# vsois/hanabi-agents

Measured on AMD Instinct MI355X. Metric: env_steps_per_sec, higher is better.
Workload: dtype u8 env/encoder + bfloat16 Q-net GEMM (fp32 accumulate, fp32 master weights)

## Files before the change

### hanabi-agents_amd/csrc/actor_fused.hip

```cpp
#include <hip/hip_runtime.h>
#include <hip/hip_bf16.h>
#include <hip/hip_fp16.h>

#include <cstdint>
#include <type_traits>

#include "../../include/hanabi_hip.h"
#include "common.hpp"
#include "env_kernel.hpp"

using hb::fail;

namespace {

typedef __bf16 bf16x8 __attribute__((ext_vector_type(8)));
typedef _Float16 f16x8 __attribute__((ext_vector_type(8)));
typedef float f32x4 __attribute__((ext_vector_type(4)));

constexpr int FM = 128;
constexpr int FH = 512;
constexpr int FNT = 512;
constexpr int FK = 51;
constexpr int S2 = FH / 32;
constexpr int LUT_BYTES = 65536;
constexpr int H_BYTES = FM * FH * 2;
constexpr int FRAG_FLOATS = 3 * 8 * FM;
constexpr int LDS_TOTAL = H_BYTES + FRAG_FLOATS * 4;
constexpr float NEG_BIG = -1e30f;

struct FusedArgs {
  const uint32_t* obs;
  long long m;
  int words;
  int s1;
  const uint4* w1f;
  const float* b1;
  const uint4* w2f;
  const float* b2;
  const float* support;
  float* q;
  int n_actions, n_pass;
  const int8_t* legal;
  int32_t* actions;
  float epsilon;
  unsigned long long seed, draw;
  long long first_gid;
  unsigned long long* stamps;
};

#ifdef HB_STAMPS
#define HB_FSTAMP(slot)                                                                              \
  do {                                                                                               \
    __builtin_amdgcn_sched_barrier(0);                                                               \
    unsigned long long hb_t_;                                                                        \
    asm volatile("s_memtime %0\n\ts_waitcnt lgkmcnt(0)" : "=s"(hb_t_)::"memory");                    \
    if (a.stamps && lane == 0) a.stamps[(static_cast<long long>(blockIdx.x) * 8 + wave) * 16 + (slot)] = hb_t_; \
    __builtin_amdgcn_sched_barrier(0);                                                               \
  } while (0)
#define HB_FSTAMP_REAL(slot)                                                                         \
  do {                                                                                               \
    unsigned long long hb_t_;                                                                        \
    asm volatile("s_memrealtime %0\n\ts_waitcnt lgkmcnt(0)" : "=s"(hb_t_)::"memory");                \
    if (a.stamps && lane == 0) a.stamps[(static_cast<long long>(blockIdx.x) * 8 + wave) * 16 + (slot)] = hb_t_; \
  } while (0)
#else
#define HB_FSTAMP(slot) do {} while (0)
#define HB_FSTAMP_REAL(slot) do {} while (0)
#endif

template <bool F16>
__device__ __forceinline__ uint32_t pack16(float lo, float hi) {
  if constexpr (F16) {
    const _Float16 a = static_cast<_Float16>(lo), b = static_cast<_Float16>(hi);
    uint16_t ua, ub;
    __builtin_memcpy(&ua, &a, 2);
    __builtin_memcpy(&ub, &b, 2);
    return static_cast<uint32_t>(ua) | (static_cast<uint32_t>(ub) << 16);
  } else {
    const __hip_bfloat16 a = __float2bfloat16(lo), b = __float2bfloat16(hi);
    return static_cast<uint32_t>(*reinterpret_cast<const uint16_t*>(&a)) |
           (static_cast<uint32_t>(*reinterpret_cast<const uint16_t*>(&b)) << 16);
  }
}
template <bool F16>
__device__ __forceinline__ uint32_t bits2_one(uint32_t b, int p) {
  const uint32_t t = (b >> (2 * p)) & 3u;
  return __umul24((t | (t << 15)) & 0x00010001u, F16 ? 0x3C00u : 0x3F80u);
}
template <bool F16>
__device__ __forceinline__ f32x4 mfma16(const uint4& wv, const uint4& xv, const f32x4& c) {
  if constexpr (F16) {
    union { uint4 u; f16x8 f; } w, x;
    w.u = wv; x.u = xv;
    return __builtin_amdgcn_mfma_f32_16x16x32_f16(w.f, x.f, c, 0, 0, 0);
  } else {
    union { uint4 u; bf16x8 f; } w, x;
    w.u = wv; x.u = xv;
    return __builtin_amdgcn_mfma_f32_16x16x32_bf16(w.f, x.f, c, 0, 0, 0);
  }
}
typedef float f32x2 __attribute__((ext_vector_type(2)));
typedef unsigned int u32x2 __attribute__((ext_vector_type(2)));
__device__ __forceinline__ float vmax(float a, float b) {
  float r;
  asm("v_max_f32 %0, %1, %2" : "=v"(r) : "v"(a), "v"(b));
  return r;
}
__device__ __forceinline__ float vmax3(float a, float b, float c) {
  float r;
  asm("v_max3_f32 %0, %1, %2, %3" : "=v"(r) : "v"(a), "v"(b), "v"(c));
  return r;
}
__device__ __forceinline__ float exp2_fast(float x) { return __builtin_amdgcn_exp2f(x); }

template <bool F16, class K, int EG>
__device__ __forceinline__ void actor_fused_body(const FusedArgs& a) {
  __shared__ __attribute__((aligned(16))) unsigned char lds[LDS_TOTAL];
  const int tid = threadIdx.x, lane = tid & 63;
  const int wave = __builtin_amdgcn_readfirstlane(tid >> 6);
  const int r = lane & 15, qd = lane >> 4;
  const long long row0 = static_cast<long long>(blockIdx.x) * FM;
  const int s1 = a.s1, G = (s1 + 3) >> 2;
  unsigned char* lutb = lds + (LDS_TOTAL - LUT_BYTES);
  const int bits_off = LDS_TOTAL - LUT_BYTES - 2048 * G;
  unsigned char* bits = lds + bits_off;
  const int m_early = bits_off >> 14;

  HB_FSTAMP_REAL(14);
  HB_FSTAMP(0);
  const uint4* w1p = a.w1f + (4 * wave) * 64 + lane;
  uint4 wa[4], wb[4];
#pragma unroll
  for (int n = 0; n < 4; ++n) wa[n] = w1p[n * 64];

  uint32_t w[4] = {0u, 0u, 0u, 0u};
  auto load_item = [&](int it) {
    const int rr = it & (FM - 1), g = it >> 7;
    long long row = row0 + rr;
    if (row >= a.m) row = a.m - 1;
    const uint32_t* src = a.obs + row * a.words + 4 * g;
#pragma unroll
    for (int i = 0; i < 4; ++i) w[i] = (4 * g + i < a.words) ? src[i] : 0u;
  };
  if (tid < FM * G) load_item(tid);
  for (int e = tid; e < 4096; e += FNT) {
    const uint32_t v = static_cast<uint32_t>(e) >> 4;
    *reinterpret_cast<uint4*>(lutb + e * 16) = make_uint4(bits2_one<F16>(v, 0), bits2_one<F16>(v, 1), bits2_one<F16>(v, 2), bits2_one<F16>(v, 3));
  }
  for (int it = tid; it < FM * G; it += FNT) {
    const int rr = it & (FM - 1), g = it >> 7;
    if (it != tid) load_item(it);
    uint32_t* dst = reinterpret_cast<uint32_t*>(bits) + (static_cast<size_t>((rr >> 4) * G + g) * 64 + (rr & 15));
#pragma unroll
    for (int qq = 0; qq < 4; ++qq) {
      const uint32_t o = ((w[0] >> (8 * qq)) & 0xFFu) | (((w[1] >> (8 * qq)) & 0xFFu) << 8) | (((w[2] >> (8 * qq)) & 0xFFu) << 16) |
                         (((w[3] >> (8 * qq)) & 0xFFu) << 24);
      dst[qq * 16] = o;
    }
  }
  HB_FSTAMP(1);
  __syncthreads();
  HB_FSTAMP(2);

  f32x4 acc[4][8];
#pragma unroll
  for (int n = 0; n < 4; ++n) {
// ... 211 lines not shown
#pragma unroll
    HB_M HB_SWAP16(tF[m], HB_ADD)
#pragma unroll
    HB_M HB_SWAP16(zs[m], HB_ADD)
#pragma unroll
    HB_M HB_SWAP16(zt[m], HB_ADD)
#pragma unroll
    HB_M HB_SWAP32(sF[m], HB_ADD)
#pragma unroll
    HB_M HB_SWAP32(tF[m], HB_ADD)
#pragma unroll
    HB_M HB_SWAP32(zs[m], HB_ADD)
#pragma unroll
    HB_M HB_SWAP32(zt[m], HB_ADD)
#pragma unroll
    HB_M { zm[m] = -nmz[m]; qF[m] = tF[m] * __builtin_amdgcn_rcpf(sF[m]) * (1.0f / FK); }
#undef HB_M
#undef HB_SWAP16
#undef HB_SWAP32
#undef HB_ADD
    if (qd == 0) {
#pragma unroll
      for (int m = 0; m < 4; ++m) {
        const long long row = row0 + 16 * (M0 + m) + r;
        if (full_ok && row < a.m) a.q[row * A + slot] = qF[m];
        fb[16 * (M0 + m) + r] = zm[m];
        fb[8 * FM + 16 * (M0 + m) + r] = zs[m];
        fb[16 * FM + 16 * (M0 + m) + r] = zt[m];
      }
    }
    __builtin_amdgcn_sched_barrier(0);
    });
    if (p < 2) HB_FSTAMP(8 + 3 * p);
    __syncthreads();
    if (tid < 2 * FM) {
      const int rr = tid & (FM - 1), g = tid >> 7;
      const int ea = full_cap + 2 * p + g;
      const long long row = row0 + rr;
      if (ea < A && row < a.m) {
        const float* f = reinterpret_cast<const float*>(lds + H_BYTES) + (4 * g) * FM + rr;
        const float m0 = f[0], m1 = f[FM], m2 = f[2 * FM], m3 = f[3 * FM];
        const float M = fmaxf(fmaxf(m0, m1), fmaxf(m2, m3));
        const float e0 = exp2_fast(m0 - M), e1 = exp2_fast(m1 - M), e2 = exp2_fast(m2 - M), e3 = exp2_fast(m3 - M);
        const float* fs = f + 8 * FM;
        const float* ft = f + 16 * FM;
        const float S = fs[0] * e0 + fs[FM] * e1 + fs[2 * FM] * e2 + fs[3 * FM] * e3;
        const float T = ft[0] * e0 + ft[FM] * e1 + ft[2 * FM] * e2 + ft[3 * FM] * e3;
        a.q[row * A + ea] = T * __builtin_amdgcn_rcpf(S) * (1.0f / FK);
      }
    }
    if (p + 1 < n_pass) __syncthreads();
    if (p < 2) HB_FSTAMP(9 + 3 * p);
  }
  if (a.legal) {
    asm volatile("s_waitcnt vmcnt(0)" ::: "memory");
    __syncthreads();
    if (tid < FM && row0 + tid < a.m) {
      const long long g = row0 + tid;
      const unsigned long long gid = static_cast<unsigned long long>(a.first_gid + g);
      uint32_t rnd[4];
      hb::philox4x32_10(static_cast<uint32_t>(a.draw), static_cast<uint32_t>(a.draw >> 32), static_cast<uint32_t>(gid),
                        static_cast<uint32_t>(gid >> 32), static_cast<uint32_t>(a.seed), static_cast<uint32_t>(a.seed >> 32), rnd);
      const float* qr = a.q + g * A;
      const int8_t* lr = a.legal + g * A;
      float best = -INFINITY;
      unsigned long long legal_mask = 0, ties = 0;
      for (int i = 0; i < A; ++i) {
        const float v = __hip_atomic_load(qr + i, __ATOMIC_RELAXED, __HIP_MEMORY_SCOPE_AGENT);
        if (lr[i] != 0) {
          legal_mask |= 1ull << i;
          if (v > best) { best = v; ties = 1ull << i; }
          else if (v == best) ties |= 1ull << i;
        }
      }
      const float u = static_cast<float>(rnd[0] >> 8) * (1.0f / 16777216.0f);
      unsigned long long pool = (u < a.epsilon) ? legal_mask : ties;
      if (pool == 0) pool = legal_mask;
      int pick = 0;
      const int c = __popcll(pool);
      if (c > 0) {
        int k = static_cast<int>(__umulhi(rnd[1], static_cast<uint32_t>(c)));
        while (k-- > 0) pool &= pool - 1;
        pick = __ffsll(static_cast<long long>(pool)) - 1;
      }
      a.actions[g] = pick;
      if constexpr (!std::is_void_v<K>) reinterpret_cast<int*>(lds + H_BYTES)[tid] = pick;
    }
  }
  if constexpr (!std::is_void_v<K>) {
    constexpr int ENV_WORDS = hb::env_lds_words<K, EG>();
    static_assert((FM / EG) * ENV_WORDS * 4 <= H_BYTES && FM / EG <= FNT / 64, "env tail: the LDS slices must fit in H");
    __syncthreads();
    if (wave < FM / EG) {
#if defined(__HIP_DEVICE_COMPILE__)
      typedef const __attribute__((address_space(4))) unsigned char KargByte;
      typedef const __attribute__((address_space(4))) hb::EnvArgs KargEnv;
      auto kargs = __builtin_amdgcn_kernarg_segment_ptr();
      asm volatile("" : "+s"(kargs));
      constexpr size_t ENV_OFF = (sizeof(FusedArgs) + alignof(hb::EnvArgs) - 1) / alignof(hb::EnvArgs) * alignof(hb::EnvArgs);
      KargEnv& env = *(KargEnv*)((KargByte*)kargs + ENV_OFF);
#else
      const hb::EnvArgs env{};
#endif
      const long long g0 = row0 + EG * wave;
      const int uid = lane < EG ? reinterpret_cast<const int*>(lds + H_BYTES)[EG * wave + lane] : 0;
      hb::env_wave_step<K, EG>(env, g0, lane, reinterpret_cast<uint32_t*>(lds) + wave * ENV_WORDS, uid, g0 / EG);
    }
  }
  HB_FSTAMP_REAL(15);
}

template <bool F16>
__global__ __launch_bounds__(FNT) void actor_fused_kernel(const FusedArgs a) {
  actor_fused_body<F16, void, 16>(a);
}

template <bool F16, class K, int EG>
__global__ __launch_bounds__(FNT) void actor_env_fused_kernel(const FusedArgs a, const hb::EnvArgs env) {
  (void)env;
  actor_fused_body<F16, K, EG>(a);
}

template <bool F16>
__global__ __launch_bounds__(FNT) void actor_fused_grouped_kernel(const FusedArgs a, const hb_fused_tile* __restrict__ tiles) {
  const hb_fused_tile& t = tiles[blockIdx.x];
  if (!t.active) return;
  FusedArgs b = a;
  b.w1f = static_cast<const uint4*>(t.w1f); b.b1 = t.b1f; b.w2f = static_cast<const uint4*>(t.w2f); b.b2 = t.b2f;
  b.support = t.support;
  b.first_gid = t.first_game_id - static_cast<long long>(blockIdx.x) * FM;
  actor_fused_body<F16, void, 16>(b);
}

struct PackArgs {
  const __hip_bfloat16* w1; int w1_ld;
  const __hip_bfloat16* b1;
  const __hip_bfloat16* w2; int w2_ld;
  const __hip_bfloat16* b2;
  int obs_len, s1, n_actions, n_pass;
  uint4* w1f; float* b1f; uint4* w2f; float* b2f;
  int chunks1, chunks2;
  int f16;
  uint16_t* w1t; int w1t_ld;
  uint16_t* w2t; int w2t_ld;
};
__device__ __forceinline__ float bias_to_float(const __hip_bfloat16* b, int i, int f16) {
  return f16 ? __half2float(reinterpret_cast<const __half*>(b)[i]) : __bfloat162float(b[i]);
}
__host__ __device__ __forceinline__ int fused_logit(int col, int n_actions, int n_pass) {
  const int slot = col >> 6, c = col & 63, n = c >> 4, q = (c >> 2) & 3, j = c & 3;
  const int r16 = 4 * n + j;
  const int full_cap = 8 * n_pass;
  int action, atom;
  if (r16 < 12 || (r16 == 12 && q < 3)) {
    action = slot < full_cap ? slot : n_actions;
    if (action >= n_actions) return -1;
    atom = r16 < 12 ? 4 * r16 + q : 48 + q;
  } else {
    const int p = slot >> 3, w = slot & 7, f = w & 3;
    action = full_cap + 2 * p + (w >> 2);
// ... 125 lines not shown
                          int32_t n_actions, int32_t n_atoms, float* q_dev, float epsilon, uint64_t seed, uint64_t draw,
                          int64_t first_game_id, int32_t* actions_dev, int32_t dtype, void* stream) {
  if (!legal_dev || !actions_dev) return fail(HB_ERR_INVALID, "null argument");
  if (n_actions > 64) return fail(HB_ERR_INVALID, "n_actions must be 1..64 for the fused selection");
  const FusedSelect sel{legal_dev, actions_dev, epsilon, seed, draw, first_game_id};
  return fused_launch(obs_bits_dev, n_rows, obs_len, w1f_dev, b1f_dev, w2f_dev, b2f_dev, support_dev, hidden, n_actions, n_atoms, q_dev,
                      nullptr, &sel, dtype, stream);
}

int hb_actor_fused_q(const uint32_t* obs_bits_dev, int64_t n_rows, int32_t obs_len, const void* w1f_dev, const float* b1f_dev,
                     const void* w2f_dev, const float* b2f_dev, const float* support_dev, int32_t hidden, int32_t n_actions, int32_t n_atoms,
                     float* q_dev, void* stream) {
  return fused_launch(obs_bits_dev, n_rows, obs_len, w1f_dev, b1f_dev, w2f_dev, b2f_dev, support_dev, hidden, n_actions, n_atoms, q_dev,
                      nullptr, nullptr, 1, stream);
}

int hb_actor_fused_act(const uint32_t* obs_bits_dev, const int8_t* legal_dev, int64_t n_rows, int32_t obs_len, const void* w1f_dev,
                       const float* b1f_dev, const void* w2f_dev, const float* b2f_dev, const float* support_dev, int32_t hidden,
                       int32_t n_actions, int32_t n_atoms, float* q_dev, float epsilon, uint64_t seed, uint64_t draw,
                       int64_t first_game_id, int32_t* actions_dev, void* stream) {
  return hb_actor_fused_act_dt(obs_bits_dev, legal_dev, n_rows, obs_len, w1f_dev, b1f_dev, w2f_dev, b2f_dev, support_dev, hidden,
                               n_actions, n_atoms, q_dev, epsilon, seed, draw, first_game_id, actions_dev, 1, stream);
}

int hb_actor_fused_act_grouped(const hb_fused_tile* tiles_dev, int64_t n_rows, const uint32_t* obs_bits_dev, const int8_t* legal_dev,
                               int32_t obs_len, int32_t hidden, int32_t n_actions, int32_t n_atoms, float* q_dev, float epsilon,
                               uint64_t seed, uint64_t draw, int32_t* actions_dev, int32_t dtype, void* stream) {
  if (dtype != 1 && dtype != 2) return fail(HB_ERR_INVALID, "dtype must be 1 (bf16) or 2 (f16)");
  if (!tiles_dev || !obs_bits_dev || !legal_dev || !q_dev || !actions_dev) return fail(HB_ERR_INVALID, "null argument");
  if (!hb_actor_fused_supported(obs_len, hidden, n_actions, n_atoms)) return fail(HB_ERR_INVALID, "shape not covered by the fused actor kernel");
  if (n_actions > 64) return fail(HB_ERR_INVALID, "n_actions must be 1..64 for the fused selection");
  if (n_rows < 0 || n_rows % FM) return fail(HB_ERR_INVALID, "n_rows (%lld) must be a multiple of %d: one tile descriptor per %d rows",
                                             static_cast<long long>(n_rows), FM, FM);
  if (n_rows / FM > 0x7fffffff) return fail(HB_ERR_INVALID, "too many tiles");
  if (n_rows == 0) return HB_OK;
  FusedArgs a{};
  a.obs = obs_bits_dev; a.m = n_rows; a.words = (obs_len + 31) / 32; a.s1 = 2 * ((obs_len + 63) / 64);
  a.q = q_dev; a.n_actions = n_actions; a.n_pass = passes_for(n_actions);
  a.legal = legal_dev; a.actions = actions_dev; a.epsilon = epsilon; a.seed = seed; a.draw = draw;
  const dim3 grid(static_cast<unsigned>(n_rows / FM));
  if (dtype == 2) hipLaunchKernelGGL(actor_fused_grouped_kernel<true>, grid, dim3(FNT), 0, static_cast<hipStream_t>(stream), a, tiles_dev);
  else hipLaunchKernelGGL(actor_fused_grouped_kernel<false>, grid, dim3(FNT), 0, static_cast<hipStream_t>(stream), a, tiles_dev);
  HB_HIP(hipGetLastError());
  return HB_OK;
}

#ifdef HB_STAMPS
int hb_actor_fused_q_stamped(const uint32_t* obs_bits_dev, int64_t n_rows, int32_t obs_len, const void* w1f_dev, const float* b1f_dev,
                             const void* w2f_dev, const float* b2f_dev, const float* support_dev, int32_t hidden, int32_t n_actions,
                             int32_t n_atoms, float* q_dev, unsigned long long* stamps_dev, void* stream) {
  return fused_launch(obs_bits_dev, n_rows, obs_len, w1f_dev, b1f_dev, w2f_dev, b2f_dev, support_dev, hidden, n_actions, n_atoms, q_dev,
                      stamps_dev, nullptr, 1, stream);
}
#endif

static int fused_args(const uint32_t* obs_bits_dev, int64_t n_rows, int32_t obs_len, const void* w1f_dev, const float* b1f_dev,
                      const void* w2f_dev, const float* b2f_dev, const float* support_dev, int32_t hidden, int32_t n_actions,
                      int32_t n_atoms, float* q_dev, unsigned long long* stamps_dev, const FusedSelect* sel, int32_t dtype, FusedArgs& a,
                      bool* launch) {
  *launch = false;
  if (dtype != 1 && dtype != 2) return fail(HB_ERR_INVALID, "dtype must be 1 (bf16) or 2 (f16)");
  if (!obs_bits_dev || !w1f_dev || !b1f_dev || !w2f_dev || !b2f_dev || !support_dev || !q_dev) return fail(HB_ERR_INVALID, "null argument");
  if (!hb_actor_fused_supported(obs_len, hidden, n_actions, n_atoms)) return fail(HB_ERR_INVALID, "shape not covered by the fused actor kernel");
  if (n_rows <= 0) return HB_OK;
  if (!aligned16(w1f_dev) || !aligned16(w2f_dev) || !aligned16(b1f_dev) || !aligned16(b2f_dev))
    return fail(HB_ERR_ALIGN, "w1f / w2f / b1f / b2f must be 16-byte aligned");
  a = FusedArgs{};
  a.obs = obs_bits_dev; a.m = n_rows; a.words = (obs_len + 31) / 32; a.s1 = 2 * ((obs_len + 63) / 64);
  a.w1f = static_cast<const uint4*>(w1f_dev); a.b1 = b1f_dev; a.w2f = static_cast<const uint4*>(w2f_dev); a.b2 = b2f_dev;
  a.support = support_dev; a.q = q_dev; a.n_actions = n_actions; a.n_pass = passes_for(n_actions);
  a.stamps = stamps_dev;
  if (sel) {
    a.legal = sel->legal; a.actions = sel->actions; a.epsilon = sel->epsilon; a.seed = sel->seed; a.draw = sel->draw;
    a.first_gid = sel->first_gid;
  }
  *launch = true;
  return HB_OK;
}

static int fused_launch(const uint32_t* obs_bits_dev, int64_t n_rows, int32_t obs_len, const void* w1f_dev, const float* b1f_dev,
                        const void* w2f_dev, const float* b2f_dev, const float* support_dev, int32_t hidden, int32_t n_actions,
                        int32_t n_atoms, float* q_dev, unsigned long long* stamps_dev, const FusedSelect* sel, int32_t dtype, void* stream) {
  FusedArgs a;
  bool go = false;
  if (int rc = fused_args(obs_bits_dev, n_rows, obs_len, w1f_dev, b1f_dev, w2f_dev, b2f_dev, support_dev, hidden, n_actions, n_atoms, q_dev,
                          stamps_dev, sel, dtype, a, &go))
    return rc;
  if (!go) return HB_OK;
  const dim3 grid(static_cast<unsigned>((n_rows + FM - 1) / FM));
  if (dtype == 2) hipLaunchKernelGGL(actor_fused_kernel<true>, grid, dim3(FNT), 0, static_cast<hipStream_t>(stream), a);
  else hipLaunchKernelGGL(actor_fused_kernel<false>, grid, dim3(FNT), 0, static_cast<hipStream_t>(stream), a);
  HB_HIP(hipGetLastError());
  return HB_OK;
}

}

namespace {

using ActEnvFull2 = hb::Cfg<2, 5, 5, 5, 8, 3>;
using ActEnvFull5 = hb::Cfg<5, 5, 5, 4, 8, 3>;
constexpr int ENV_EG = 16;

template <class K>
static bool is_cfg(const hb::EnvVariant& v) {
  return v.P == K::P && v.C == K::C && v.R == K::R && v.H == K::H && v.INFO == K::INFO && v.LIFE == K::LIFE;
}

template <bool F16, class K>
static void launch_act_env(const FusedArgs& a, const hb::EnvArgs& env, dim3 grid, hipStream_t stream) {
  if (env.ev_start && env.ev_stop)
    hipExtLaunchKernelGGL((actor_env_fused_kernel<F16, K, ENV_EG>), grid, dim3(FNT), 0, stream, env.ev_start, env.ev_stop, 0, a, env);
  else
    hipLaunchKernelGGL((actor_env_fused_kernel<F16, K, ENV_EG>), grid, dim3(FNT), 0, stream, a, env);
}

}

namespace hb {

bool actor_env_fused_supported(const EnvVariant& v) { return is_cfg<ActEnvFull2>(v) || is_cfg<ActEnvFull5>(v); }

int actor_env_fused_launch(const uint32_t* obs_bits_dev, const int8_t* legal_dev, int64_t n_rows, int32_t obs_len, const void* w1f_dev,
                           const float* b1f_dev, const void* w2f_dev, const float* b2f_dev, const float* support_dev, int32_t hidden,
                           int32_t n_actions, int32_t n_atoms, float* q_dev, float epsilon, uint64_t seed, uint64_t draw,
                           int64_t first_game_id, int32_t* actions_dev, int32_t dtype, const EnvArgs& env, const EnvVariant& var,
                           void* stream) {
  if (!legal_dev || !actions_dev) return fail(HB_ERR_INVALID, "null argument");
  if (!actor_env_fused_supported(var)) return fail(HB_ERR_INVALID, "no fused policy + env kernel for this game configuration");
  if (n_rows != env.n) return fail(HB_ERR_INVALID, "n_rows (%lld) must equal the env's game count (%lld)", static_cast<long long>(n_rows), env.n);
  if (n_actions != var.n_actions || obs_len != var.obs_len) return fail(HB_ERR_INVALID, "actor shape does not match the env");
  const FusedSelect sel{legal_dev, actions_dev, epsilon, seed, draw, first_game_id};
  FusedArgs a;
  bool go = false;
  if (int rc = fused_args(obs_bits_dev, n_rows, obs_len, w1f_dev, b1f_dev, w2f_dev, b2f_dev, support_dev, hidden, n_actions, n_atoms, q_dev,
                          nullptr, &sel, dtype, a, &go))
    return rc;
  if (!go) return HB_OK;
  const dim3 grid(static_cast<unsigned>((n_rows + FM - 1) / FM));
  const hipStream_t st = static_cast<hipStream_t>(stream);
  const bool f16 = dtype == 2;
  if (is_cfg<ActEnvFull2>(var)) {
    if (f16) launch_act_env<true, ActEnvFull2>(a, env, grid, st);
    else launch_act_env<false, ActEnvFull2>(a, env, grid, st);
  } else {
    if (f16) launch_act_env<true, ActEnvFull5>(a, env, grid, st);
    else launch_act_env<false, ActEnvFull5>(a, env, grid, st);
  }
  HB_HIP(hipGetLastError());
  return HB_OK;
}

}
```

### hanabi-agents_amd/csrc/env_api.hip

```cpp
#include <hip/hip_runtime.h>

#include <cstdarg>
#include <cstdio>
#include <cstdlib>
#include <cstring>
#include <new>
#include <string>
#include <vector>

#include "../../include/hanabi_hip.h"
#include "common.hpp"
#include "env_kernel.hpp"

namespace hb {
const EnvVariant* variants_full(int* n);
const EnvVariant* variants_small(int* n);
const EnvVariant* variants_vsmall(int* n);

thread_local std::string g_error;
int fail(int code, const char* fmt, ...) {
  char buf[512];
  va_list ap;
  va_start(ap, fmt);
  vsnprintf(buf, sizeof buf, fmt, ap);
// ... 435 lines not shown
                       float* reward_dev, int8_t* terminal_dev, float* agent_reward_dev, int8_t* agent_step_type_dev,
                       int8_t* score_dev, void* stream) {
  if (!e) return fail(HB_ERR_INVALID, "null env");
  if (!actions_dev) return fail(HB_ERR_INVALID, "actions_dev is required");
  if (int rc = check_out_packed(obs_bits_dev, obs_dev, legal_dev)) return rc;
  hb::EnvArgs a{};
  a.mode = hb::MODE_STEP;
  a.actions = actions_dev;
  a.obs = obs_dev;
  a.obs_bits = obs_bits_dev;
  a.legal = legal_dev;
  a.reward = reward_dev;
  a.terminal = terminal_dev;
  a.agent_reward = agent_reward_dev;
  a.agent_step_type = agent_step_type_dev;
  a.score = score_dev;
  if (int rc = join_refill(e, stream)) return rc;
  if (int rc = launch(e, a, stream)) return rc;
  return refill_async(e, stream);
}

int hb_env_step_select_packed(hb_env* e, const float* q_dev, const int8_t* sel_legal_dev, float epsilon, uint64_t seed, uint64_t draw,
                              int64_t first_game_id, int32_t* actions_out_dev, uint32_t* obs_bits_dev, int8_t* obs_dev,
                              int8_t* legal_dev, float* reward_dev, int8_t* terminal_dev, float* agent_reward_dev,
                              int8_t* agent_step_type_dev, int8_t* score_dev, void* stream) {
  if (!e) return fail(HB_ERR_INVALID, "null env");
  if (!q_dev || !sel_legal_dev || !actions_out_dev) return fail(HB_ERR_INVALID, "q_dev, sel_legal_dev and actions_out_dev are required");
  if ((reinterpret_cast<uintptr_t>(q_dev) & 15) || (reinterpret_cast<uintptr_t>(sel_legal_dev) & 3))
    return fail(HB_ERR_ALIGN, "q_dev must be 16-byte and sel_legal_dev 4-byte aligned");
  if (e->var->n_actions > 64) return fail(HB_ERR_INVALID, "the fused selection handles at most 64 actions");
  if (int rc = check_out_packed(obs_bits_dev, obs_dev, legal_dev)) return rc;
  hb::EnvArgs a{};
  a.mode = hb::MODE_STEP;
  a.sel_q = q_dev;
  a.sel_legal = sel_legal_dev;
  a.sel_actions = actions_out_dev;
  a.sel_eps = epsilon;
  a.sel_seed = seed;
  a.sel_draw = draw;
  a.sel_first_gid = first_game_id;
  a.obs = obs_dev;
  a.obs_bits = obs_bits_dev;
  a.legal = legal_dev;
  a.reward = reward_dev;
  a.terminal = terminal_dev;
  a.agent_reward = agent_reward_dev;
  a.agent_step_type = agent_step_type_dev;
  a.score = score_dev;
  if (int rc = join_refill(e, stream)) return rc;
  if (int rc = launch(e, a, stream)) return rc;
  return refill_async(e, stream);
}

int hb_actor_fused_act_step(hb_env* e, const uint32_t* obs_bits_dev, const int8_t* legal_dev, int64_t n_rows, int32_t obs_len,
                            const void* w1f_dev, const float* b1f_dev, const void* w2f_dev, const float* b2f_dev, const float* support_dev,
                            int32_t hidden, int32_t n_actions, int32_t n_atoms, float* q_dev, float epsilon, uint64_t seed, uint64_t draw,
                            int64_t first_game_id, int32_t* actions_dev, int32_t dtype, uint32_t* obs_bits_out_dev, int8_t* legal_out_dev,
                            float* reward_dev, int8_t* terminal_dev, float* agent_reward_dev, int8_t* agent_step_type_dev,
                            int8_t* score_dev, void* stream) {
  if (!e) return fail(HB_ERR_INVALID, "null env");
  if (e->shuffled) return fail(HB_ERR_INVALID, "the fused policy + env kernel has no colour-permuted form: step a shuffled env with "
                                               "hb_env_step_packed or hb_env_step_select_packed");
  if (int rc = check_out_packed(obs_bits_out_dev, nullptr, legal_out_dev)) return rc;
  hb::EnvArgs a{};
  a.mode = hb::MODE_STEP;
  a.obs_bits = obs_bits_out_dev;
  a.legal = legal_out_dev;
  a.reward = reward_dev;
  a.terminal = terminal_dev;
  a.agent_reward = agent_reward_dev;
  a.agent_step_type = agent_step_type_dev;
  a.score = score_dev;
  prepare(e, a);
  if (int rc = join_refill(e, stream)) return rc;
  if (int rc = hb::actor_env_fused_launch(obs_bits_dev, legal_dev, n_rows, obs_len, w1f_dev, b1f_dev, w2f_dev, b2f_dev, support_dev, hidden,
                                          n_actions, n_atoms, q_dev, epsilon, seed, draw, first_game_id, actions_dev, dtype, a, *e->var,
                                          stream))
    return rc;
  return refill_async(e, stream);
}

int hb_actor_fused_step_supported(const hb_env* e) { return e && !e->shuffled && hb::actor_env_fused_supported(*e->var) ? 1 : 0; }

#ifdef HB_STAMPS
int hb_env_step_stamped(hb_env* e, const int32_t* actions_dev, int8_t* obs_dev, int8_t* legal_dev,
                        unsigned long long* stamps_dev, void* stream) {
  hb::EnvArgs a{};
  a.mode = hb::MODE_STEP;
  a.actions = actions_dev;
  a.obs = obs_dev;
  a.legal = legal_dev;
  a.stamps = stamps_dev;
  if (int rc = join_refill(e, stream)) return rc;
  if (int rc = launch(e, a, stream)) return rc;
  return refill_async(e, stream);
}
#endif

int hb_env_illegal_count(hb_env* e, int64_t* out) {
  if (!e || !out) return fail(HB_ERR_INVALID, "null argument");
  unsigned long long v = 0;
  HB_HIP(hipMemcpy(&v, e->illegal, 8, hipMemcpyDeviceToHost));
  *out = static_cast<int64_t>(v);
  return HB_OK;
}

int hb_env_stats(hb_env* e, int64_t* episodes, int64_t* score_sum) {
  if (!e || !episodes || !score_sum) return fail(HB_ERR_INVALID, "null argument");
  std::vector<unsigned long long> v(static_cast<size_t>(2 * e->stat_slots));
  HB_HIP(hipMemcpy(v.data(), e->illegal + 1, 16 * e->stat_slots, hipMemcpyDeviceToHost));
  unsigned long long ep = 0, sc = 0;
  for (long long i = 0; i < e->stat_slots; ++i) { ep += v[2 * i]; sc += v[2 * i + 1]; }
  *episodes = static_cast<int64_t>(ep);
  *score_sum = static_cast<int64_t>(sc);
  return HB_OK;
}

int hb_env_set_refill_period(hb_env* e, int32_t steps) {
  if (!e) return fail(HB_ERR_INVALID, "null env");
  if (steps < 1 || steps > e->cfg.max_life) return fail(HB_ERR_INVALID, "refill period must be 1..max_life (%d)", e->cfg.max_life);
  e->refill_period = steps;
  return HB_OK;
}

int hb_env_set_async_refill(hb_env* e, int32_t on) {
  if (!e) return fail(HB_ERR_INVALID, "null env");
  HB_HIP(hipDeviceSynchronize());
  e->refill_in_flight = false;
  e->async_refill = on != 0;
  return HB_OK;
}

int hb_env_export_state(hb_env* e, uint32_t* rows_dev, void* stream) {
  if (!e || !rows_dev) return fail(HB_ERR_INVALID, "null argument");
  HB_HIP(hipMemcpyAsync(rows_dev, e->state, static_cast<size_t>(e->n) * e->var->state_words * 4, hipMemcpyDeviceToDevice,
                        static_cast<hipStream_t>(stream)));
  return HB_OK;
// ... 72 lines not shown
```

### hanabi-agents_amd/csrc/env_kernel.hpp

```cpp
#pragma once
#include <hip/hip_runtime.h>
#include <hip/hip_ext.h>
#include <stdint.h>
#include <utility>

struct hb_config;

namespace hb {

enum { MODE_STEP = 0, MODE_OBSERVE = 1, MODE_RESET = 2 };
constexpr int NEXT_DECK_BYTES = 64;
enum { MV_PLAY = 0, MV_DISCARD = 1, MV_RCOLOR = 2, MV_RRANK = 3 };

struct EnvArgs {
  uint32_t* state;
  const int32_t* actions;
  const uint8_t* mask;
  const uint8_t* decks;
  uint8_t* next_deck;
  uint8_t* refill;
  int8_t* obs;
  uint32_t* obs_bits;
  int8_t* legal;
  float* reward;
// ... 356 lines not shown
      dv |= ((disc >> (c * K::CPC)) & ((1ull << K::CPC) - 1ull)) << (K::CPC * sig(c));
    });
    acc.template put64<K::DISC_OFF, K::D>(dv);
  } else {
    acc.template put64<K::DISC_OFF, K::D>(disc);
  }
  {
    const uint32_t valid = w2 & 1u;
    const int la_player = (w2 >> 1) & 7, la_type = (w2 >> 4) & 3, la_ci = (w2 >> 6) & 7, la_toff = (w2 >> 9) & 7;
    const int la_color_t = (w2 >> 12) & 7, la_rank = (w2 >> 15) & 7;
    const int la_color = SHUF ? sig(la_color_t) : la_color_t;
    const uint32_t la_scored = (w2 >> 18) & 1u, la_info = (w2 >> 19) & 1u, la_mask = (w2 >> 20) & 31u;
    int actor = la_player - o;
    if (actor < 0) actor += P;
    int target = actor + la_toff;
    if (target >= P) target -= P;
    const uint32_t reveal = valid & static_cast<uint32_t>(la_type >= MV_RCOLOR);
    const uint32_t cardmv = valid & static_cast<uint32_t>(la_type <= MV_DISCARD);
    const uint32_t is_rc = valid & static_cast<uint32_t>(la_type == MV_RCOLOR);
    const uint32_t is_rr = valid & static_cast<uint32_t>(la_type == MV_RRANK);
    const uint32_t is_play = valid & static_cast<uint32_t>(la_type == MV_PLAY);
    constexpr int o1 = K::LA_OFF, o2 = o1 + P, o3 = o2 + 4, o4 = o3 + P, o5 = o4 + C, o6 = o5 + R, o7 = o6 + H,
                  o8 = o7 + H, o9 = o8 + K::BITS;
    acc.template put<o1, P>(valid << actor);
    acc.template put<o2, 4>(valid << la_type);
    acc.template put<o3, P>(reveal << target);
    acc.template put<o4, C>(is_rc << la_color);
    acc.template put<o5, R>(is_rr << la_rank);
    acc.template put<o6, H>(reveal ? la_mask : 0u);
    acc.template put<o7, H>(cardmv << la_ci);
    acc.template put<o8, K::BITS>(cardmv << (la_color * R + la_rank));
    acc.template put<o9, 2>((is_play & la_scored) | ((is_play & la_info) << 1));
  }
  static_for<P>([&](auto REL) {
    constexpr int rel = decltype(REL)::value;
    int p = o + rel;
    if (p >= P) p -= P;
    const int n_p = hand_n(p);
    const uint64_t kn = (static_cast<uint64_t>(row[K::W_KNOW + 2 * p + 1]) << 32) | row[K::W_KNOW + 2 * p];
    static_for<H>([&](auto I) {
      constexpr int i = decltype(I)::value;
      const uint32_t k = static_cast<uint32_t>(kn >> (12 * i)) & 0xFFFu;
      const uint32_t cp = seen_colours<SHUF, C>(k & 31u, sg), rp = (k >> 5) & 31u;
      const uint32_t plaus = __umul24(spread_colors<C, R>(cp), rp);
      const uint32_t ch = (k >> 10) & 1u, rh = (k >> 11) & 1u;
      uint64_t v = plaus | (static_cast<uint64_t>(ch ? cp : 0u) << K::BITS) |
                   (static_cast<uint64_t>(rh ? rp : 0u) << (K::BITS + C));
      if (i >= n_p) v = 0;
      acc.template put64<K::KN_OFF + (rel * H + i) * K::KN_SLOT, K::KN_SLOT>(v);
    });
  });
}

template <class K, int G, bool SHUF = false>
__device__ __forceinline__ void env_wave_step(const EnvArgs& a, long long g0, int lane, uint32_t* const srow, int uid_in,
                                              long long wslot) {
  constexpr int P = K::P, C = K::C, R = K::R, H = K::H;
  constexpr int LPG = 1;
  uint32_t* const obits = srow + G * K::SWP;
  uint32_t* const lbits = obits + G * K::NWP;
  const long long left = a.n - g0;
  const int nvalid = left <= 0 ? 0 : (left < G ? static_cast<int>(left) : G);
  const int mode = a.mode;
  HB_STAMP_REAL(10);
  HB_STAMP(0);

  const bool active = lane < nvalid && lane < G;
  const long long gi = g0 + lane;
  bool mask_in = true;
  uint4 nd[4] = {make_uint4(0u, 0u, 0u, 0u), make_uint4(0u, 0u, 0u, 0u), make_uint4(0u, 0u, 0u, 0u), make_uint4(0u, 0u, 0u, 0u)};
  const uint4* const ndp = reinterpret_cast<const uint4*>(a.next_deck + gi * NEXT_DECK_BYTES);
  if (active) {
    if (mode == MODE_RESET && a.mask) mask_in = a.mask[gi] != 0;
    if (mode == MODE_RESET && mask_in) {
      nd[0] = ndp[0]; nd[1] = ndp[1]; nd[2] = ndp[2]; nd[3] = ndp[3];
    }
  }
  uint4 pm = make_uint4(0u, 0u, 0u, 0u);
  if constexpr (SHUF) {
    if (active) pm = reinterpret_cast<const uint4*>(a.perms)[gi];
  }

  {
    constexpr int Q = K::SW / 4;
    constexpr int ROUNDS = (G * Q + 63) / 64;
    const uint4* src = reinterpret_cast<const uint4*>(a.state + g0 * K::SW);
    uint4 v[ROUNDS];
#pragma unroll
    for (int r = 0; r < ROUNDS; ++r) {
      const int e = lane + 64 * r;
      v[r] = e < nvalid * Q ? src[e] : make_uint4(0u, 0u, 0u, 0u);
    }
#pragma unroll
    for (int r = 0; r < ROUNDS; ++r) {
      const int e = lane + 64 * r;
      if (e < nvalid * Q) {
        const int g = e / Q, q = e - g * Q;
        uint32_t* d = srow + g * K::SWP + 4 * q;
        d[0] = v[r].x; d[1] = v[r].y; d[2] = v[r].z; d[3] = v[r].w;
      }
    }
  }
  HB_STAMP(1);
  wave_sync();
  HB_STAMP(2);

  uint32_t* const row = srow + lane * K::SWP;
  uint32_t w0 = 0, w1 = 0, w2 = 0, w3 = 0, w6 = 0;
  uint64_t accw = 0, disc = 0;
  float out_reward = 0.f;
  int out_term = 0, out_score = 0;
  bool illegal = false, need_reset = false, keep_seats = true;
  int reset_start = 0;

  auto hand_n = [&](int p) -> int { return (w1 >> (15 + 3 * p)) & 7; };
  auto fw = [&](int c) -> int { return (w1 >> (3 * c)) & 7; };
  auto score_now = [&]() -> int {
    if (((w0 >> 10) & 7) == 0) return 0;
    int s = 0;
#pragma unroll
    for (int c = 0; c < C; ++c) s += fw(c);
    return s;
  };

  if (active) {
    w0 = row[0]; w1 = row[1]; w2 = row[2]; w3 = row[3]; w6 = row[6];
    accw = (static_cast<uint64_t>(row[5]) << 32) | row[4];
    disc = (static_cast<uint64_t>(row[9]) << 32) | row[8];
    if (mode == MODE_RESET) {
      need_reset = mask_in;
      keep_seats = false;
      reset_start = a.start_player;
    } else if (mode == MODE_STEP && ((w0 >> 19) & 3) == 0) {
      {
        int fsum = 0;
#pragma unroll
        for (int c = 0; c < C; ++c) fsum += fw(c);
        if (((w0 >> 10) & 7) <= 1 || (w0 & 63) == 0 || fsum >= C * R - 1) {
          nd[0] = ndp[0]; nd[1] = ndp[1]; nd[2] = ndp[2]; nd[3] = ndp[3];
        }
      }
      if constexpr (SHUF) {
        const int xc0 = uid_in - 2 * H;
        if (xc0 >= 0 && xc0 < (P - 1) * C) {
          const uint32_t sgm = perm_of(pm, (w0 >> 13) & 7);
          const int tgt = xc0 / C, seen = xc0 - tgt * C;
          int c = 0;
#pragma unroll
          for (int k = 0; k < C; ++k) c = static_cast<int>((sgm >> (3 * k)) & 7u) == seen ? k : c;
          uid_in = 2 * H + tgt * C + c;
        }
      }
// ... 396 lines not shown
    for (int i = 0; i < K::NW; ++i) ob[i] = acc.w[i];
#pragma unroll
    for (int i = K::NW; i < K::NWP; ++i) ob[i] = 0;
    uint32_t* lb = lbits + lane * K::LW;
    lb[0] = static_cast<uint32_t>(legal);
    lb[1] = static_cast<uint32_t>(legal >> 32);
    lb[2] = 0;
  }
  wave_sync();
  if (a.obs_bits) {
    uint32_t* dst = a.obs_bits + g0 * K::NW;
    for (int e = lane; e < nvalid * K::NW; e += 64) {
      const int g = e / K::NW, i = e - g * K::NW;
      dst[e] = obits[g * K::NWP + i];
    }
  }
  if (a.obs) expand_rows<K::OBS_LEN>(obits, K::NWP, nvalid, a.obs + g0 * K::OBS_LEN, lane);
  if (a.legal) expand_rows<K::A>(lbits, K::LW, nvalid, a.legal + g0 * K::A, lane);
}

template <class K, int G>
void launch_encode(const EncodeArgs& a, hipStream_t stream) {
  const long long per_block = 4LL * G;
  const unsigned blocks = static_cast<unsigned>((a.n + per_block - 1) / per_block);
  if (blocks == 0) return;
  hipLaunchKernelGGL((encode_rows_kernel<K, G>), dim3(blocks), dim3(256), 0, stream, a);
}

using LaunchFn = void (*)(const EnvArgs&, hipStream_t);
using EncodeFn = void (*)(const EncodeArgs&, hipStream_t);
struct EnvVariant {
  int P, C, R, H, INFO, LIFE;
  int obs_len, n_actions, deck, state_words;
  LaunchFn g8, g16, g32, g64, refill;
  LaunchFn s8, s16, s32, s64;
  EncodeFn e16, e32;
};

template <class K>
constexpr EnvVariant make_variant() {
  return EnvVariant{K::P, K::C, K::R, K::H, K::INFO, K::LIFE, K::OBS_LEN, K::A, K::D, K::SW,
                    &launch_env<K, 8>, &launch_env<K, 16>, &launch_env<K, 32>, &launch_env<K, 64>, &launch_refill<K>,
                    &launch_env_shuf<K, 8>, &launch_env_shuf<K, 16>, &launch_env_shuf<K, 32>, &launch_env_shuf<K, 64>,
                    &launch_encode<K, 16>, &launch_encode<K, 32>};
}

const EnvVariant* find_variant(const ::hb_config* c);

bool actor_env_fused_supported(const EnvVariant& v);
int actor_env_fused_launch(const uint32_t* obs_bits_dev, const int8_t* legal_dev, int64_t n_rows, int32_t obs_len, const void* w1f_dev,
                           const float* b1f_dev, const void* w2f_dev, const float* b2f_dev, const float* support_dev, int32_t hidden,
                           int32_t n_actions, int32_t n_atoms, float* q_dev, float epsilon, uint64_t seed, uint64_t draw,
                           int64_t first_game_id, int32_t* actions_dev, int32_t dtype, const EnvArgs& env, const EnvVariant& var,
                           void* stream);

}
```

Measured before the change: 313.8 million.

## Spread action selection across all waves and prefetch env state rows early

Action selection used to run on one thread per row over 128 rows with scalar atomic loads. It now runs on 16 lanes per wave across all 8 waves. Legal masks are preloaded before the barrier, Q values are read as vectorised buffer loads, and the argmax/tie loop is fully unrolled and branch-free. The env state rows are requested right after the barrier so that load overlaps selection, and each wave steps its own games with its own pick, which removes the LDS handoff of picks and the extra __syncthreads. The costs are higher register pressure (qv[64], lw[16] and the prefetched rows) and a hard requirement that EG equal 16. Stamped entry points are also added for profiling.

```diff
diff --git a/hanabi-agents_amd/csrc/actor_fused.hip b/hanabi-agents_amd/csrc/actor_fused.hip
--- a/hanabi-agents_amd/csrc/actor_fused.hip
+++ b/hanabi-agents_amd/csrc/actor_fused.hip
@@ -49,19 +49,20 @@
 };
 
 #ifdef HB_STAMPS
+constexpr int FSTAMP_SLOTS = 24;
 #define HB_FSTAMP(slot)                                                                              \
   do {                                                                                               \
     __builtin_amdgcn_sched_barrier(0);                                                               \
     unsigned long long hb_t_;                                                                        \
     asm volatile("s_memtime %0\n\ts_waitcnt lgkmcnt(0)" : "=s"(hb_t_)::"memory");                    \
-    if (a.stamps && lane == 0) a.stamps[(static_cast<long long>(blockIdx.x) * 8 + wave) * 16 + (slot)] = hb_t_; \
+    if (a.stamps && lane == 0) a.stamps[(static_cast<long long>(blockIdx.x) * 8 + wave) * FSTAMP_SLOTS + (slot)] = hb_t_; \
     __builtin_amdgcn_sched_barrier(0);                                                               \
   } while (0)
 #define HB_FSTAMP_REAL(slot)                                                                         \
   do {                                                                                               \
     unsigned long long hb_t_;                                                                        \
     asm volatile("s_memrealtime %0\n\ts_waitcnt lgkmcnt(0)" : "=s"(hb_t_)::"memory");                \
-    if (a.stamps && lane == 0) a.stamps[(static_cast<long long>(blockIdx.x) * 8 + wave) * 16 + (slot)] = hb_t_; \
+    if (a.stamps && lane == 0) a.stamps[(static_cast<long long>(blockIdx.x) * 8 + wave) * FSTAMP_SLOTS + (slot)] = hb_t_; \
   } while (0)
 #else
 #define HB_FSTAMP(slot) do {} while (0)
@@ -101,6 +102,7 @@
 }
 typedef float f32x2 __attribute__((ext_vector_type(2)));
 typedef unsigned int u32x2 __attribute__((ext_vector_type(2)));
+typedef unsigned int u32x4 __attribute__((ext_vector_type(4)));
 __device__ __forceinline__ float vmax(float a, float b) {
   float r;
   asm("v_max_f32 %0, %1, %2" : "=v"(r) : "v"(a), "v"(b));
@@ -112,6 +114,20 @@
   return r;
 }
 __device__ __forceinline__ float exp2_fast(float x) { return __builtin_amdgcn_exp2f(x); }
+
+#if defined(__HIP_DEVICE_COMPILE__)
+typedef const __attribute__((address_space(4))) hb::EnvArgs EnvKarg;
+__device__ __forceinline__ EnvKarg* env_kernarg() {
+  typedef const __attribute__((address_space(4))) unsigned char KargByte;
+  auto kargs = __builtin_amdgcn_kernarg_segment_ptr();
+  asm volatile("" : "+s"(kargs));
+  constexpr size_t ENV_OFF = (sizeof(FusedArgs) + alignof(hb::EnvArgs) - 1) / alignof(hb::EnvArgs) * alignof(hb::EnvArgs);
+  return (EnvKarg*)((KargByte*)kargs + ENV_OFF);
+}
+#else
+typedef const hb::EnvArgs EnvKarg;
+__device__ __forceinline__ EnvKarg* env_kernarg() { return nullptr; }
+#endif
 
 template <bool F16, class K, int EG>
 __device__ __forceinline__ void actor_fused_body(const FusedArgs& a) {
@@ -429,60 +445,122 @@
     if (p + 1 < n_pass) __syncthreads();
     if (p < 2) HB_FSTAMP(9 + 3 * p);
   }
+  HB_FSTAMP(16);
+  constexpr int SG = 16;
+  static_assert(std::is_void_v<K> || EG == SG, "the selecting lane is the lane that steps the game");
+  const long long g0 = row0 + SG * wave;
+  const bool sel = a.legal && lane < SG && g0 + lane < a.m;
+  std::conditional_t<std::is_void_v<K>, int, hb::EnvRows<K, EG>> erows;
+  uint32_t rnd[4] = {0u, 0u, 0u, 0u};
+  uint32_t lw[16];
+  if (sel) {
+    const int8_t* lr = a.legal + (g0 + lane) * A;
+    if ((A & 3) == 0 && (reinterpret_cast<uintptr_t>(a.legal) & 3u) == 0) {
+      hb::static_for<16>([&](auto J) {
+        constexpr int j = decltype(J)::value;
+        if (4 * j < A) lw[j] = reinterpret_cast<const uint32_t*>(lr)[j];
+      });
+    } else {
+      uint32_t lb[64];
+      hb::static_for<16>([&](auto J) {
+        constexpr int j = decltype(J)::value;
+        if (4 * j < A) {
+#pragma unroll
+          for (int k = 0; k < 4; ++k) lb[4 * j + k] = static_cast<uint8_t>(lr[4 * j + k < A ? 4 * j + k : A - 1]);
+        }
+      });
+      hb::static_for<16>([&](auto J) {
+        constexpr int j = decltype(J)::value;
+        if (4 * j < A) {
+          uint32_t w4 = 0u;
+#pragma unroll
+          for (int k = 0; k < 4; ++k) w4 |= (4 * j + k < A ? lb[4 * j + k] : 0u) << (8 * k);
+          lw[j] = w4;
+        }
+      });
+    }
+  }
+  int pick = 0;
   if (a.legal) {
     asm volatile("s_waitcnt vmcnt(0)" ::: "memory");
     __syncthreads();
-    if (tid < FM && row0 + tid < a.m) {
-      const long long g = row0 + tid;
-      const unsigned long long gid = static_cast<unsigned long long>(a.first_gid + g);
-      uint32_t rnd[4];
+    HB_FSTAMP(17);
+    if constexpr (!std::is_void_v<K>) {
+      EnvKarg* const env = env_kernarg();
+      hb::env_rows_request<K, EG>(env->state, env->n, g0, lane, erows);
+    } else {
+      (void)erows;
+    }
+    if (sel) {
+      float qv[64];
+      const long long left = a.m - g0;
+      const int nrec = (left < SG ? static_cast<int>(left) : SG) * A * 4;
+      const __amdgpu_buffer_rsrc_t qrs = __builtin_amdgcn_make_buffer_rsrc(a.q + g0 * A, 0, nrec, 0x00020000);
+      constexpr int SC1 = 16;
+      const int voff = lane * A * 4;
+      if ((A & 3) == 0 && (reinterpret_cast<uintptr_t>(a.q) & 15u) == 0) {
+        hb::static_for<16>([&](auto J) {
+          constexpr int j = decltype(J)::value;
+          if (4 * j < A) {
+            const u32x4 t = __builtin_amdgcn_raw_buffer_load_b128(qrs, voff + 16 * j, 0, SC1);
+            qv[4 * j] = __uint_as_float(t.x); qv[4 * j + 1] = __uint_as_float(t.y);
+            qv[4 * j + 2] = __uint_as_float(t.z); qv[4 * j + 3] = __uint_as_float(t.w);
+          }
+        });
+      } else {
+        hb::static_for<16>([&](auto J) {
+          constexpr int j = decltype(J)::value;
+          if (4 * j < A) {
+#pragma unroll
+            for (int k = 0; k < 4; ++k) qv[4 * j + k] = __uint_as_float(__builtin_amdgcn_raw_buffer_load_b32(qrs, voff + 4 * (4 * j + k), 0, SC1));
+          }
+        });
+      }
+      const unsigned long long gid = static_cast<unsigned long long>(a.first_gid + g0 + lane);
       hb::philox4x32_10(static_cast<uint32_t>(a.draw), static_cast<uint32_t>(a.draw >> 32), static_cast<uint32_t>(gid),
                         static_cast<uint32_t>(gid >> 32), static_cast<uint32_t>(a.seed), static_cast<uint32_t>(a.seed >> 32), rnd);
-      const float* qr = a.q + g * A;
-      const int8_t* lr = a.legal + g * A;
+      asm volatile("" : "+v"(rnd[0]), "+v"(rnd[1]));
       float best = -INFINITY;
-      unsigned long long legal_mask = 0, ties = 0;
-      for (int i = 0; i < A; ++i) {
-        const float v = __hip_atomic_load(qr + i, __ATOMIC_RELAXED, __HIP_MEMORY_SCOPE_AGENT);
-        if (lr[i] != 0) {
-          legal_mask |= 1ull << i;
-          if (v > best) { best = v; ties = 1ull << i; }
-          else if (v == best) ties |= 1ull << i;
+      uint32_t lm[2] = {0u, 0u}, ti[2] = {0u, 0u};
+      hb::static_for<16>([&](auto J) {
+        constexpr int j = decltype(J)::value;
+        if (4 * j < A) {
+          hb::static_for<4>([&](auto KK) {
+            constexpr int k = decltype(KK)::value, i = 4 * j + k, h = i >> 5;
+            constexpr uint32_t bit = 1u << (i & 31);
+            const float v = qv[i];
+            const bool leg = (lw[j] & (0xFFu << (8 * k))) != 0;
+            const bool gt = leg && v > best, eq = leg && v == best;
+            lm[h] |= leg ? bit : 0u;
+            ti[h] = gt ? bit : (eq ? (ti[h] | bit) : ti[h]);
+            if constexpr (h == 1) ti[0] = gt ? 0u : ti[0];
+            best = gt ? v : best;
+          });
         }
-      }
+      });
+      const unsigned long long legal_mask = (static_cast<unsigned long long>(lm[1]) << 32) | lm[0];
+      const unsigned long long ties = (static_cast<unsigned long long>(ti[1]) << 32) | ti[0];
       const float u = static_cast<float>(rnd[0] >> 8) * (1.0f / 16777216.0f);
       unsigned long long pool = (u < a.epsilon) ? legal_mask : ties;
       if (pool == 0) pool = legal_mask;
-      int pick = 0;
       const int c = __popcll(pool);
       if (c > 0) {
         int k = static_cast<int>(__umulhi(rnd[1], static_cast<uint32_t>(c)));
         while (k-- > 0) pool &= pool - 1;
         pick = __ffsll(static_cast<long long>(pool)) - 1;
       }
-      a.actions[g] = pick;
-      if constexpr (!std::is_void_v<K>) reinterpret_cast<int*>(lds + H_BYTES)[tid] = pick;
-    }
+      a.actions[g0 + lane] = pick;
+    }
+    HB_FSTAMP(18);
   }
   if constexpr (!std::is_void_v<K>) {
     constexpr int ENV_WORDS = hb::env_lds_words<K, EG>();
-    static_assert((FM / EG) * ENV_WORDS * 4 <= H_BYTES && FM / EG <= FNT / 64, "env tail: the LDS slices must fit in H");
-    __syncthreads();
-    if (wave < FM / EG) {
-#if defined(__HIP_DEVICE_COMPILE__)
-      typedef const __attribute__((address_space(4))) unsigned char KargByte;
-      typedef const __attribute__((address_space(4))) hb::EnvArgs KargEnv;
-      auto kargs = __builtin_amdgcn_kernarg_segment_ptr();
-      asm volatile("" : "+s"(kargs));
-      constexpr size_t ENV_OFF = (sizeof(FusedArgs) + alignof(hb::EnvArgs) - 1) / alignof(hb::EnvArgs) * alignof(hb::EnvArgs);
-      KargEnv& env = *(KargEnv*)((KargByte*)kargs + ENV_OFF);
-#else
-      const hb::EnvArgs env{};
-#endif
-      const long long g0 = row0 + EG * wave;
-      const int uid = lane < EG ? reinterpret_cast<const int*>(lds + H_BYTES)[EG * wave + lane] : 0;
-      hb::env_wave_step<K, EG>(env, g0, lane, reinterpret_cast<uint32_t*>(lds) + wave * ENV_WORDS, uid, g0 / EG);
-    }
+    static_assert((FM / EG) * ENV_WORDS * 4 <= H_BYTES && FM / EG == FNT / 64, "env tail: the LDS slices must fit in H");
+    HB_FSTAMP(19);
+    EnvKarg* const env = env_kernarg();
+    if (!a.legal) hb::env_rows_request<K, EG>(env->state, env->n, g0, lane, erows);
+    hb::env_wave_step<K, EG>(*env, g0, lane, reinterpret_cast<uint32_t*>(lds) + wave * ENV_WORDS, pick, g0 / EG, &erows);
+    HB_FSTAMP(20);
   }
   HB_FSTAMP_REAL(15);
 }
@@ -714,6 +792,16 @@
   return fused_launch(obs_bits_dev, n_rows, obs_len, w1f_dev, b1f_dev, w2f_dev, b2f_dev, support_dev, hidden, n_actions, n_atoms, q_dev,
                       stamps_dev, nullptr, 1, stream);
 }
+int hb_actor_fused_act_stamped(const uint32_t* obs_bits_dev, const int8_t* legal_dev, int64_t n_rows, int32_t obs_len, const void* w1f_dev,
+                               const float* b1f_dev, const void* w2f_dev, const float* b2f_dev, const float* support_dev, int32_t hidden,
+                               int32_t n_actions, int32_t n_atoms, float* q_dev, float epsilon, uint64_t seed, uint64_t draw,
+                               int64_t first_game_id, int32_t* actions_dev, unsigned long long* stamps_dev, void* stream) {
+  if (!legal_dev || !actions_dev) return fail(HB_ERR_INVALID, "null argument");
+  if (n_actions > 64) return fail(HB_ERR_INVALID, "n_actions must be 1..64 for the fused selection");
+  const FusedSelect sel{legal_dev, actions_dev, epsilon, seed, draw, first_game_id};
+  return fused_launch(obs_bits_dev, n_rows, obs_len, w1f_dev, b1f_dev, w2f_dev, b2f_dev, support_dev, hidden, n_actions, n_atoms, q_dev,
+                      stamps_dev, &sel, 1, stream);
+}
 #endif
 
 static int fused_args(const uint32_t* obs_bits_dev, int64_t n_rows, int32_t obs_len, const void* w1f_dev, const float* b1f_dev,
@@ -787,7 +875,7 @@
                            const float* b1f_dev, const void* w2f_dev, const float* b2f_dev, const float* support_dev, int32_t hidden,
                            int32_t n_actions, int32_t n_atoms, float* q_dev, float epsilon, uint64_t seed, uint64_t draw,
                            int64_t first_game_id, int32_t* actions_dev, int32_t dtype, const EnvArgs& env, const EnvVariant& var,
-                           void* stream) {
+                           void* stream, unsigned long long* stamps_dev) {
   if (!legal_dev || !actions_dev) return fail(HB_ERR_INVALID, "null argument");
   if (!actor_env_fused_supported(var)) return fail(HB_ERR_INVALID, "no fused policy + env kernel for this game configuration");
   if (n_rows != env.n) return fail(HB_ERR_INVALID, "n_rows (%lld) must equal the env's game count (%lld)", static_cast<long long>(n_rows), env.n);
@@ -796,7 +884,7 @@
   FusedArgs a;
   bool go = false;
   if (int rc = fused_args(obs_bits_dev, n_rows, obs_len, w1f_dev, b1f_dev, w2f_dev, b2f_dev, support_dev, hidden, n_actions, n_atoms, q_dev,
-                          nullptr, &sel, dtype, a, &go))
+                          stamps_dev, &sel, dtype, a, &go))
     return rc;
   if (!go) return HB_OK;
   const dim3 grid(static_cast<unsigned>((n_rows + FM - 1) / FM));
diff --git a/hanabi-agents_amd/csrc/env_api.hip b/hanabi-agents_amd/csrc/env_api.hip
--- a/hanabi-agents_amd/csrc/env_api.hip
+++ b/hanabi-agents_amd/csrc/env_api.hip
@@ -511,12 +511,12 @@
   return refill_async(e, stream);
 }
 
-int hb_actor_fused_act_step(hb_env* e, const uint32_t* obs_bits_dev, const int8_t* legal_dev, int64_t n_rows, int32_t obs_len,
-                            const void* w1f_dev, const float* b1f_dev, const void* w2f_dev, const float* b2f_dev, const float* support_dev,
-                            int32_t hidden, int32_t n_actions, int32_t n_atoms, float* q_dev, float epsilon, uint64_t seed, uint64_t draw,
-                            int64_t first_game_id, int32_t* actions_dev, int32_t dtype, uint32_t* obs_bits_out_dev, int8_t* legal_out_dev,
-                            float* reward_dev, int8_t* terminal_dev, float* agent_reward_dev, int8_t* agent_step_type_dev,
-                            int8_t* score_dev, void* stream) {
+static int fused_act_step(hb_env* e, const uint32_t* obs_bits_dev, const int8_t* legal_dev, int64_t n_rows, int32_t obs_len,
+                          const void* w1f_dev, const float* b1f_dev, const void* w2f_dev, const float* b2f_dev, const float* support_dev,
+                          int32_t hidden, int32_t n_actions, int32_t n_atoms, float* q_dev, float epsilon, uint64_t seed, uint64_t draw,
+                          int64_t first_game_id, int32_t* actions_dev, int32_t dtype, uint32_t* obs_bits_out_dev, int8_t* legal_out_dev,
+                          float* reward_dev, int8_t* terminal_dev, float* agent_reward_dev, int8_t* agent_step_type_dev,
+                          int8_t* score_dev, unsigned long long* actor_stamps_dev, unsigned long long* env_stamps_dev, void* stream) {
   if (!e) return fail(HB_ERR_INVALID, "null env");
   if (e->shuffled) return fail(HB_ERR_INVALID, "the fused policy + env kernel has no colour-permuted form: step a shuffled env with "
                                                "hb_env_step_packed or hb_env_step_select_packed");
@@ -530,18 +530,40 @@
   a.agent_reward = agent_reward_dev;
   a.agent_step_type = agent_step_type_dev;
   a.score = score_dev;
+  a.stamps = env_stamps_dev;
   prepare(e, a);
   if (int rc = join_refill(e, stream)) return rc;
   if (int rc = hb::actor_env_fused_launch(obs_bits_dev, legal_dev, n_rows, obs_len, w1f_dev, b1f_dev, w2f_dev, b2f_dev, support_dev, hidden,
                                           n_actions, n_atoms, q_dev, epsilon, seed, draw, first_game_id, actions_dev, dtype, a, *e->var,
-                                          stream))
+                                          stream, actor_stamps_dev))
     return rc;
   return refill_async(e, stream);
 }
 
+int hb_actor_fused_act_step(hb_env* e, const uint32_t* obs_bits_dev, const int8_t* legal_dev, int64_t n_rows, int32_t obs_len,
+                            const void* w1f_dev, const float* b1f_dev, const void* w2f_dev, const float* b2f_dev, const float* support_dev,
+                            int32_t hidden, int32_t n_actions, int32_t n_atoms, float* q_dev, float epsilon, uint64_t seed, uint64_t draw,
+                            int64_t first_game_id, int32_t* actions_dev, int32_t dtype, uint32_t* obs_bits_out_dev, int8_t* legal_out_dev,
+                            float* reward_dev, int8_t* terminal_dev, float* agent_reward_dev, int8_t* agent_step_type_dev,
+                            int8_t* score_dev, void* stream) {
+  return fused_act_step(e, obs_bits_dev, legal_dev, n_rows, obs_len, w1f_dev, b1f_dev, w2f_dev, b2f_dev, support_dev, hidden, n_actions,
+                        n_atoms, q_dev, epsilon, seed, draw, first_game_id, actions_dev, dtype, obs_bits_out_dev, legal_out_dev, reward_dev,
+                        terminal_dev, agent_reward_dev, agent_step_type_dev, score_dev, nullptr, nullptr, stream);
+}
+
 int hb_actor_fused_step_supported(const hb_env* e) { return e && !e->shuffled && hb::actor_env_fused_supported(*e->var) ? 1 : 0; }
 
 #ifdef HB_STAMPS
+int hb_actor_fused_act_step_stamped(hb_env* e, const uint32_t* obs_bits_dev, const int8_t* legal_dev, int64_t n_rows, int32_t obs_len,
+                                    const void* w1f_dev, const float* b1f_dev, const void* w2f_dev, const float* b2f_dev,
+                                    const float* support_dev, int32_t hidden, int32_t n_actions, int32_t n_atoms, float* q_dev, float epsilon,
+                                    uint64_t seed, uint64_t draw, int64_t first_game_id, int32_t* actions_dev, uint32_t* obs_bits_out_dev,
+                                    int8_t* legal_out_dev, float* reward_dev, int8_t* terminal_dev, int8_t* score_dev,
+                                    unsigned long long* actor_stamps_dev, unsigned long long* env_stamps_dev, void* stream) {
+  return fused_act_step(e, obs_bits_dev, legal_dev, n_rows, obs_len, w1f_dev, b1f_dev, w2f_dev, b2f_dev, support_dev, hidden, n_actions,
+                        n_atoms, q_dev, epsilon, seed, draw, first_game_id, actions_dev, 1, obs_bits_out_dev, legal_out_dev, reward_dev,
+                        terminal_dev, nullptr, nullptr, score_dev, actor_stamps_dev, env_stamps_dev, stream);
+}
 int hb_env_step_stamped(hb_env* e, const int32_t* actions_dev, int8_t* obs_dev, int8_t* legal_dev,
                         unsigned long long* stamps_dev, void* stream) {
   hb::EnvArgs a{};
diff --git a/hanabi-agents_amd/csrc/env_kernel.hpp b/hanabi-agents_amd/csrc/env_kernel.hpp
--- a/hanabi-agents_amd/csrc/env_kernel.hpp
+++ b/hanabi-agents_amd/csrc/env_kernel.hpp
@@ -432,9 +432,27 @@
   });
 }
 
+template <class K, int G>
+struct EnvRows {
+  static constexpr int Q = K::SW / 4, ROUNDS = (G * Q + 63) / 64;
+  uint4 v[ROUNDS];
+};
+template <class K, int G>
+__device__ __forceinline__ void env_rows_request(const uint32_t* state, long long n, long long g0, int lane, EnvRows<K, G>& rows) {
+  constexpr int Q = EnvRows<K, G>::Q;
+  const long long left = n - g0;
+  const int nvalid = left <= 0 ? 0 : (left < G ? static_cast<int>(left) : G);
+  const uint4* src = reinterpret_cast<const uint4*>(state + g0 * K::SW);
+#pragma unroll
+  for (int r = 0; r < EnvRows<K, G>::ROUNDS; ++r) {
+    const int e = lane + 64 * r;
+    rows.v[r] = e < nvalid * Q ? src[e] : make_uint4(0u, 0u, 0u, 0u);
+  }
+}
+
 template <class K, int G, bool SHUF = false>
 __device__ __forceinline__ void env_wave_step(const EnvArgs& a, long long g0, int lane, uint32_t* const srow, int uid_in,
-                                              long long wslot) {
+                                              long long wslot, const EnvRows<K, G>* pre = nullptr) {
   constexpr int P = K::P, C = K::C, R = K::R, H = K::H;
   constexpr int LPG = 1;
   uint32_t* const obits = srow + G * K::SWP;
@@ -462,22 +480,17 @@
   }
 
   {
-    constexpr int Q = K::SW / 4;
-    constexpr int ROUNDS = (G * Q + 63) / 64;
-    const uint4* src = reinterpret_cast<const uint4*>(a.state + g0 * K::SW);
-    uint4 v[ROUNDS];
-#pragma unroll
-    for (int r = 0; r < ROUNDS; ++r) {
-      const int e = lane + 64 * r;
-      v[r] = e < nvalid * Q ? src[e] : make_uint4(0u, 0u, 0u, 0u);
-    }
-#pragma unroll
-    for (int r = 0; r < ROUNDS; ++r) {
+    constexpr int Q = EnvRows<K, G>::Q;
+    EnvRows<K, G> rows;
+    if (pre) rows = *pre;
+    else env_rows_request<K, G>(a.state, a.n, g0, lane, rows);
+#pragma unroll
+    for (int r = 0; r < EnvRows<K, G>::ROUNDS; ++r) {
       const int e = lane + 64 * r;
       if (e < nvalid * Q) {
         const int g = e / Q, q = e - g * Q;
         uint32_t* d = srow + g * K::SWP + 4 * q;
-        d[0] = v[r].x; d[1] = v[r].y; d[2] = v[r].z; d[3] = v[r].w;
+        d[0] = rows.v[r].x; d[1] = rows.v[r].y; d[2] = rows.v[r].z; d[3] = rows.v[r].w;
       }
     }
   }
@@ -980,6 +993,6 @@
                            const float* b1f_dev, const void* w2f_dev, const float* b2f_dev, const float* support_dev, int32_t hidden,
                            int32_t n_actions, int32_t n_atoms, float* q_dev, float epsilon, uint64_t seed, uint64_t draw,
                            int64_t first_game_id, int32_t* actions_dev, int32_t dtype, const EnvArgs& env, const EnvVariant& var,
-                           void* stream);
-
-}
+                           void* stream, unsigned long long* stamps_dev = nullptr);
+
+}
```

Result: faster. 317.1 million (median of 5 runs) (+1.0%).
